# fgarciacardenas/SplaTAM

Hardware: AMD Instinct MI355X
Metric: rasterize fwd+bwd frames/sec @640×480, 300k Gaussians; HBM GB/s vs peak (higher is better)
Workload: dtype f32

## Files before the change

### splatam_amd/csrc/gsr_backward.hip

```cpp
#include <cstdlib>
#include <utility>

#include "gsr_chain.h"
#include "gsr_diag.h"
#include "gsr_glue_common.h"
#include "gsr_render_fwd.h"

namespace gsr {

template <bool OPAC>
__device__ __forceinline__ void pair_geom(float* vk, float araw, float dLa, float G, v2f d) {
    if constexpr (OPAC) {
        const v2f ho = v2f{araw, G} * dLa;
        const v2f hv = ho.x * d;
        const v2f hh = hv.x * d;
        vk[0] = hv.x;
        vk[1] = hv.y;
        vk[2] = hh.x;
        vk[3] = hh.y;
        vk[4] = hv.y * d.y;
        vk[5] = ho.y;
        return;
    }
    const v2f hv = (araw * dLa) * d;
// ... 370 lines not shown
                    e[k].dx = d[k].x;
                    e[k].dy = d[k].y;
                    e[k].xx = d[k].x * d[k].x;
                    e[k].xy = d[k].x * d[k].y;
                    e[k].yy = d[k].y * d[k].y;
                    e[k].o2 = o * o;
                    e[k].c2 = dch[k] * dch[k];
                    const float hc = h * dch[k];
                    e[k].hc[0] = hc * dp0;
                    e[k].hc[1] = hc * dp1;
                    e[k].hc[2] = hc * dp2;
                }
                mom_pass<MOM, 0, 4>(e, mdp2, mdpp, lane, dst);
                mom_pass<MOM, 4, 4>(e, mdp2, mdpp, lane, dst);
                mom_pass<MOM, 8, 4>(e, mdp2, mdpp, lane, dst);
                if constexpr (MOM == 1) {
                    mom_pass<MOM, 12, 4>(e, mdp2, mdpp, lane, dst);
                } else {
                    mom_pass<MOM, 12, 4>(e, mdp2, mdpp, lane, dst);
                    mom_pass<MOM, 16, 4>(e, mdp2, mdpp, lane, dst);
                    mom_pass<MOM, 20, 4>(e, mdp2, mdpp, lane, dst);
                    mom_pass<MOM, 24, 5>(e, mdp2, mdpp, lane, dst);
                    mom_pass<MOM, 29, 5>(e, mdp2, mdpp, lane, dst);
                }
            } else if constexpr (NV <= 6) {
                float v[4 * NV];
#pragma unroll
                for (int k = 0; k < 4; k++) {
                    pair_geom<OPAC>(v + NV * k, araw[k], dLa[k], G[k], d[k]);
                    pair_colours<COL1, COL2, Q2, C1>(v + NV * k + O_C1, dch[k], dp01, dp2, dq0, dq01, dq2);
                }
                if constexpr (kAblate == 1) {
#pragma unroll
                    for (int q = 0; q < 4 * NV; q++) ablate_sink += v[q];
                } else {
                    reduce_store<NV>(v, lane, dst, true);
                }
            } else {
                constexpr int NA = 5 + (OPAC ? 1 : 0), NB = NV - NA;
                {
                    float v[4 * NA];
#pragma unroll
                    for (int k = 0; k < 4; k++) pair_geom<OPAC>(v + NA * k, araw[k], dLa[k], G[k], d[k]);
                    reduce_store<NA>(v, lane, dst, true);
                }
                {
                    float v[4 * NB];
#pragma unroll
                    for (int k = 0; k < 4; k++) {
                        pair_colours<COL1, COL2, Q2, C1>(v + NB * k, dch[k], dp01, dp2, dq0, dq01, dq2);
                    }
                    reduce_store<NB>(v, lane, dst + NA, true);
                }
            }
        }
        dg.phase(3);
        __syncthreads();
        dg.phase(4);
        constexpr int TPE = TILE_PIX / BB, NQ = (NV + TPE - 1) / TPE, NQR = (RS + TPE - 1) / TPE;
        int t_ = tid;
        asm volatile("" : "+v"(t_));
        const int e = t_ / TPE, q = t_ % TPE;
        if (kAblate != 2 && e < cnt) {
            float c[NQ];
#pragma unroll
            for (int i = 0; i < NQ; i++) c[i] = 0.f;
            const int nb = __popc((uint32_t)s_mask[e]);
            float* src = s_acc + (int)s_base[e] * NV;
            for (int b = 0; b < nb; b++, src += NV) {
#pragma unroll
                for (int i = 0; i < NQ; i++)
                    if (q + TPE * i < NV) {
                        c[i] += src[q + TPE * i];
                        if constexpr (!kBulkClear) src[q + TPE * i] = 0.f;
                    }
            }
            float* dst = inst + (size_t)RS * s_u[e];
#pragma unroll
            for (int i = 0; i < NQR; i++)
                if (q + TPE * i < RS) {
                    const float val = i < NQ ? c[i] : 0.f;
                    dst[q + TPE * i] = val;
                }
        }
        dg.phase(5);
        __syncthreads();
        if constexpr (kBulkClear) {
            const int used = cnt > 0 ? (int)s_base[cnt - 1] + __popc((uint32_t)s_mask[cnt - 1]) : 0;
            float4* const a4 = reinterpret_cast<float4*>(s_acc);
            const float4 z = make_float4(0.f, 0.f, 0.f, 0.f);
            for (int q4 = tid; q4 < (used * NV + 3) / 4; q4 += TILE_PIX) a4[q4] = z;
        }
        dg.phase(6);
        dg.batch();
        hi -= cnt;
    }
    if (kAblate == 1 && ablate_sink == 1.2345f) inst[0] = ablate_sink;
}

template <bool DUAL, bool OPAC, bool COL1, bool COL2, int Q2 = 3, int MOM = 0>
__global__ void __launch_bounds__(TILE_PIX, (bwd_waves<DUAL, OPAC, COL1, COL2, Q2, MOM>()))
render_bwd_kernel(Camera cam, const uint2* __restrict__ ranges, const PointEntry* __restrict__ point_list,
                  const float4* __restrict__ rr, const uint32_t* __restrict__ blocksums,
                  const float* __restrict__ final_T,
                  const uint32_t* __restrict__ n_contrib, const float* __restrict__ dL_dpix,
                  const float* __restrict__ dL_dpix2, float* __restrict__ inst, BwdGuard guard,
                  unsigned long long* clk) {
    kclock_begin(clk);
    RenderDiag dg;
    dg.begin();
    if (guard.overflow()) {
        kclock_end(clk);
        return;
    }
    __shared__ __attribute__((aligned(16))) char smem[BwdShape<DUAL, OPAC, COL1, COL2, Q2, MOM>::bytes];
    const int tid = threadIdx.x;
    const int tile = sched_tile(cam), tx = tile % cam.gx, ty = tile / cam.gx;
    dg.tile(tile);
    const int px = tx * TILE_X + tile_px(tid);
    const int py = ty * TILE_Y + tile_py(tid);
    const bool inside = px < cam.W && py < cam.H;
    const int pid = py * cam.W + px;
    const int HW = cam.W * cam.H;
    BwdPix pin{0.f, 0u, 0.f, 0.f, 0.f, 0.f, 0.f, 0.f};
    if (inside) {
        pin.T_final = final_T[pid];
        pin.last = n_contrib[pid];
        pin.dp0 = dL_dpix[pid];
        pin.dp1 = dL_dpix[HW + pid];
        pin.dp2 = dL_dpix[2 * HW + pid];
        if (DUAL) {
            pin.dq0 = dL_dpix2[pid];
            if (Q2 == 3) {
                pin.dq1 = dL_dpix2[HW + pid];
                pin.dq2 = dL_dpix2[2 * HW + pid];
            }
        }
    }
    if constexpr (!DUAL && COL1 && MOM == 0) {
        if (!__syncthreads_or(pin.dp1 != 0.f || pin.dp2 != 0.f)) {
            bwd_tile<DUAL, OPAC, COL1, COL2, Q2, MOM, 1>(cam, tile, pin, ranges, point_list, rr, blocksums, inst, guard,
                                                         smem, dg);
            dg.end();
            kclock_end(clk);
            return;
        }
    }
    bwd_tile<DUAL, OPAC, COL1, COL2, Q2, MOM>(cam, tile, pin, ranges, point_list, rr, blocksums, inst, guard, smem, dg);
    dg.end();
    kclock_end(clk);
}

constexpr size_t track_lds_bytes() {
    return FwdShape<true>::bytes > BwdShape<true, false, false, true, 1, 0>::bytes
               ? FwdShape<true>::bytes
               : BwdShape<true, false, false, true, 1, 0>::bytes;
}
template <bool IMAGES>
__global__ void __launch_bounds__(TILE_PIX, 5)
render_track_kernel(Camera cam, const uint2* __restrict__ ranges, PointEntry* __restrict__ point_list,
                    uint64_t* __restrict__ keys, const float4* __restrict__ rr, const uint32_t* __restrict__ blocksums,
                    float* __restrict__ final_T, uint32_t* __restrict__ n_contrib, float* __restrict__ out_color,
                    float* __restrict__ out_color2, float* __restrict__ out_depth, SpecGuard guard,
                    unsigned long long* clk, TrackL1 l1, float* __restrict__ inst) {
    kclock_begin(clk);
    RenderDiag dg;
    dg.begin();
    if (guard.overflow()) {
        kclock_end(clk);
        return;
    }
    __shared__ __attribute__((aligned(16))) char smem[track_lds_bytes()];
    if constexpr (!IMAGES) {
        final_T = nullptr;
        cam.rowmax = nullptr;
    }
    const int tile = sched_tile(cam);
    dg.tile(tile);
    const FwdPix f = fwd_tile<true>(cam, tile, ranges, point_list, keys, rr, guard, smem, dg);
    float grad[4];
    constexpr bool kStoreGrads = false;
    static_assert(!kStoreGrads, "render_track_kernel's callers pass no gradient images");
    fwd_epilogue<true, true, kStoreGrads>(cam, tile, f, final_T, n_contrib, out_color, out_color2, out_depth, l1,
                                          grad);
    __syncthreads();
    const BwdPix pin{f.T, f.last16 >> 4, grad[0], grad[1], grad[2], grad[3], 0.f, 0.f};
    Camera cb = cam;
    cb.rowmax = nullptr;
    bwd_tile<true, false, false, true, 1, 0>(cb, tile, pin, ranges, point_list, rr, blocksums, inst,
                                             BwdGuard{guard.counters, guard.cap_inst}, smem, dg);
    dg.end();
    kclock_end(clk);
}

int track_records_stride() { return BwdShape<true, false, false, true, 1, 0>::RS; }

hipError_t launch_render_track(const Camera& cam, const uint2* ranges, uint64_t* point_list, uint64_t* keys,
                               GeomPtrs geo, float* final_T, uint32_t* n_contrib, float* out_color,
                               float* out_color2, float* out_depth, SpecGuard guard, const TrackL1& l1, float* inst,
                               hipStream_t s, unsigned long long* clk) {
    auto k = final_T != nullptr ? render_track_kernel<true> : render_track_kernel<false>;
    hipLaunchKernelGGL(k, dim3(cam.gx * cam.gy), dim3(TILE_PIX), 0, s, cam, ranges, point_list,
                       keys, geo.rr, geo.blocksums, final_T, n_contrib, out_color, out_color2, out_depth, guard, clk,
                       l1, inst);
    return hipGetLastError();
}

template <bool DUAL, bool OPAC, bool COL1, bool COL2, int Q2 = 3>
static auto bwd_variant() { return render_bwd_kernel<DUAL, OPAC, COL1, COL2, Q2>; }

RecLayout bwd_rec_layout(unsigned need, bool dual) {
    const bool op = need & NEED_OPACITY, c1 = need & NEED_COLORS, c2 = dual && (need & NEED_COLORS2);
    const int q2 = (dual && (need & NEED_DL2_CH0_ONLY)) ? 1 : 3;
    RecLayout L;
    int nv = 5;
    L.o_op = op ? nv : -1;
    nv += op ? 1 : 0;
    L.o_c1 = c1 ? nv : -1;
    nv += c1 ? 3 : 0;
    L.o_c2 = c2 ? nv : -1;
    L.n_c2 = c2 ? q2 : 0;
    nv += L.n_c2;
    L.stride = (nv + 1) & ~1;
    return L;
}

hipError_t launch_render_bwd(const Camera& cam, const uint2* ranges, const uint64_t* point_list, GeomPtrs geo,
                             const float* final_T, const uint32_t* n_contrib, const float* dL_dpix,
                             const float* colors2, const float* dL_dpix2, unsigned need, float* inst,
                             BwdGuard guard, hipStream_t s, unsigned long long* clk) {
    const bool op = need & NEED_OPACITY, c1 = need & NEED_COLORS, c2 = colors2 && (need & NEED_COLORS2);
    const bool q1 = need & NEED_DL2_CH0_ONLY;
    auto k = bwd_variant<false, true, true, false>();
    if (!colors2) {
        k = op ? (c1 ? bwd_variant<false, 1, 1, 0>() : bwd_variant<false, 1, 0, 0>())
               : (c1 ? bwd_variant<false, 0, 1, 0>() : bwd_variant<false, 0, 0, 0>());
    } else if (q1 && !op && !c1) {
        k = c2 ? bwd_variant<true, 0, 0, 1, 1>() : bwd_variant<true, 0, 0, 0, 1>();
    } else if (q1) {
        k = op ? (c1 ? (c2 ? bwd_variant<true, 1, 1, 1, 1>() : bwd_variant<true, 1, 1, 0, 1>())
                     : (c2 ? bwd_variant<true, 1, 0, 1, 1>() : bwd_variant<true, 1, 0, 0, 1>()))
               : (c2 ? bwd_variant<true, 0, 1, 1, 1>() : bwd_variant<true, 0, 1, 0, 1>());
    } else {
        k = op ? (c1 ? (c2 ? bwd_variant<true, 1, 1, 1>() : bwd_variant<true, 1, 1, 0>())
                     : (c2 ? bwd_variant<true, 1, 0, 1>() : bwd_variant<true, 1, 0, 0>()))
               : (c1 ? (c2 ? bwd_variant<true, 0, 1, 1>() : bwd_variant<true, 0, 1, 0>())
                     : (c2 ? bwd_variant<true, 0, 0, 1>() : bwd_variant<true, 0, 0, 0>()));
    }
    hipLaunchKernelGGL(k, dim3(cam.gx * cam.gy), dim3(TILE_PIX), 0, s, cam, ranges, point_list, geo.rr, geo.blocksums,
                       final_T, n_contrib, dL_dpix, dL_dpix2, inst, guard, clk);
    return hipGetLastError();
}

template <bool POSE, bool SHL>
__device__ __forceinline__ void gauss_bwd_body(Camera cam, GaussIn g, GeomPtrs geo, const int* __restrict__ radii,
                                               const float* __restrict__ inst, RecLayout rec, GradsOut out,
                                               BwdGuard guard, PoseFuse pf) {
    if constexpr (!SHL) {
        g.shs = nullptr;
        g.M = 0;
    }
    const int i = blockIdx.x * blockDim.x + threadIdx.x;
    if (!POSE && i >= g.P) return;
    const bool live = i < g.P;
    const int nsh = g.shs ? (cam.sh_degree + 1) * (cam.sh_degree + 1) : 0;
    float g2[9] = {0.f, 0.f, 0.f, 0.f, 0.f, 0.f, 0.f, 0.f, 0.f};
    float dcol2[3] = {0.f, 0.f, 0.f};
    float dmean[3] = {0.f, 0.f, 0.f}, dcov[6] = {0.f, 0.f, 0.f, 0.f, 0.f, 0.f}, dscale[3] = {0.f, 0.f, 0.f},
          drot[4] = {0.f, 0.f, 0.f, 0.f};
    float dsh[48];
#pragma unroll
    for (int k = 0; k < 48; k++) dsh[k] = 0.f;
    GaussGeom gg;
    gg.m = make_float3(0.f, 0.f, 0.f);
    gg.s = make_float3(0.f, 0.f, 0.f);
    gg.q = make_float4(0.f, 0.f, 0.f, 0.f);
    const int rad = live ? radii[i] : 0;
    const bool xf_geom = POSE && pf.ls;
    TrackXf x;
    x.mw = pf.means_world; x.ur = pf.unnorm_rot; x.ls = pf.ls; x.scols = pf.scols;
    XfRaw xr{};
    if (xf_geom && live) xr = track_xform_load(x, i, false);
    uint32_t off = 0, cnt = 0, tl = 0xFFFFFFFFu;
    if (POSE && live && rad > 0) {
        off = geo.offsets[i];
        cnt = geo.tiles[i];
        tl = reinterpret_cast<const uint32_t*>(geo.bin)[4 * (size_t)i + 3];
    }
    __shared__ Pose s_pose;
    if constexpr (POSE) {
        if (pf.ls || pf.scols != 1) {
            if (threadIdx.x == 0) s_pose = make_pose(pf.cam_q, pf.cam_t, pf.qs);
            __syncthreads();
        }
    }
    if (live && (POSE || rad > 0)) {
        if (xf_geom) {
            const Pose ps = s_pose;
            float m[3], sv[3];
            track_xform_geom_raw(xr, x.scols, ps, m, gg.q, sv);
            gg.m = make_float3(m[0], m[1], m[2]);
            gg.s = make_float3(sv[0], sv[1], sv[2]);
        } else {
            gg = load_geom(g, i);
        }
    }
    if (live && rad > 0 && !guard.overflow()) {
        if (!POSE) {
            off = geo.offsets[i];
            cnt = geo.tiles[i];
            tl = reinterpret_cast<const uint32_t*>(geo.bin)[4 * (size_t)i + 3];
        }
        float acc[INST_REC_MAX];
#pragma unroll
        for (int m = 0; m < INST_REC_MAX; m++) acc[m] = 0.f;
        const int np = rec.stride / 2;
        constexpr int RU = 4;
        for (uint32_t e0 = 0; e0 < cnt; e0 += RU) {
            float2 v[RU][INST_REC_MAX / 2];
#pragma unroll
            for (int k = 0; k < RU; k++) {
                const float2* r = reinterpret_cast<const float2*>(inst + (size_t)rec.stride * (off + e0 + k));
#pragma unroll
                for (int m = 0; m < INST_REC_MAX / 2; m++)
                    v[k][m] = (m < np && e0 + k < cnt && tile_live(tl, e0 + k)) ? r[m] : make_float2(0.f, 0.f);
            }
#pragma unroll
            for (int k = 0; k < RU; k++)
                if (e0 + k < cnt && tile_live(tl, e0 + k)) {
#pragma unroll
                    for (int m = 0; m < INST_REC_MAX / 2; m++)
                        if (m < np) {
// ... 379 lines not shown
```

### splatam_amd/csrc/gsr_capi.hip

```cpp
#include <cstdio>
#include <cstdlib>
#include <cstring>
#include <algorithm>
#include <atomic>
#include <string>

#include "../../include/gsr.h"
#include "../../include/gsr_glue.h"
#include "gsr_host.h"

using namespace gsr;

namespace {
thread_local std::string g_last_error;

__global__ void zero_words_kernel(uint32_t* __restrict__ p, size_t n) {
    for (size_t k = blockIdx.x * (size_t)blockDim.x + threadIdx.x; k < n; k += (size_t)gridDim.x * blockDim.x) p[k] = 0u;
}
std::atomic<int> g_cus[kMaxDevices];
}

namespace gsr {
int fail(int code, const std::string& msg) {
    g_last_error = msg;
// ... 53 lines not shown
    uint32_t* p = nullptr;
    uint32_t* dp = nullptr;
    hipEvent_t ev = nullptr;
    ~Pinned() {
        if (p) (void)hipHostFree(p);
        if (ev) (void)hipEventDestroy(ev);
    }
    int ensure(int dev) {
        hipError_t e;
        if (!p) {
            if ((e = hipHostMalloc((void**)&p, 32,
                                   hipHostMallocMapped | hipHostMallocCoherent | hipHostMallocPortable)) != hipSuccess)
                return hip_fail(e, "hipHostMalloc");
            if ((e = hipHostGetDevicePointer((void**)&dp, p, 0)) != hipSuccess)
                return hip_fail(e, "hipHostGetDevicePointer");
        }
        if (!ev) {
            int cur = 0;
            (void)hipGetDevice(&cur);
            if (cur != dev) (void)hipSetDevice(dev);
            e = hipEventCreateWithFlags(&ev, hipEventDisableTiming);
            if (cur != dev) (void)hipSetDevice(cur);
            if (e != hipSuccess) return hip_fail(e, "hipEventCreate");
        }
        return GSR_OK;
    }
};
thread_local Pinned g_pinned[kMaxDevices];
const bool g_snap_copy = getenv("GSR_SNAP_COPY") && atoi(getenv("GSR_SNAP_COPY")) != 0;
struct RatioHint {
    std::atomic<double> v{3.0};
};
RatioHint g_inst_ratio[kMaxDevices];

Camera make_camera(const gsr_settings* s) {
    Camera c;
    c.W = s->image_width;
    c.H = s->image_height;
    c.tan_fovx = s->tan_fovx;
    c.tan_fovy = s->tan_fovy;
    c.focal_y = (float)c.H / (2.0f * s->tan_fovy);
    c.focal_x = (float)c.W / (2.0f * s->tan_fovx);
    c.gx = (c.W + TILE_X - 1) / TILE_X;
    c.gy = (c.H + TILE_Y - 1) / TILE_Y;
    c.view = s->viewmatrix;
    c.proj = s->projmatrix;
    c.campos = s->campos;
    c.bg = s->bg;
    c.scale_modifier = s->scale_modifier;
    c.sh_degree = s->sh_degree;
    c.prefiltered = s->prefiltered;
    return c;
}

GaussIn make_gauss(const gsr_gaussians* g) {
    GaussIn o;
    o.P = g->P;
    o.M = g->shs ? g->M : 0;
    o.means3D = g->means3D;
    o.shs = (g->shs && g->M > 0) ? g->shs : nullptr;
    o.colors = g->colors_precomp;
    o.opacities = g->opacities;
    o.scales = g->scales;
    o.rotations = g->rotations;
    o.cov3D = g->cov3D_precomp;
    o.colors2 = nullptr;
    o.sh_staged = 0;
    o.alive = nullptr;
    return o;
}

int validate(const gsr_settings* s, const gsr_gaussians* g, bool forward) {
    if (!s || !g) return fail(GSR_ERR_INVALID_ARG, "null settings or gaussians");
    if (g->P < 0) return fail(GSR_ERR_INVALID_ARG, "P must be >= 0");
    if (s->binning != GSR_BINNING_CULLED && s->binning != GSR_BINNING_REFERENCE)
        return fail(GSR_ERR_INVALID_ARG, "settings.binning must be GSR_BINNING_CULLED or GSR_BINNING_REFERENCE");
    if (s->image_width <= 0 || s->image_height <= 0) return fail(GSR_ERR_INVALID_ARG, "image size must be positive");
    if (s->image_width > 16 * 65535 || s->image_height > 16 * 65535)
        return fail(GSR_ERR_INVALID_ARG, "image too large for 16-bit tile coordinates");
    if (g->P == 0) return GSR_OK;
    if (!g->means3D) return fail(GSR_ERR_INVALID_ARG, "means3D is required");
    if (forward && !g->opacities) return fail(GSR_ERR_INVALID_ARG, "opacities are required");
    if (!s->viewmatrix || !s->projmatrix || !s->bg) return fail(GSR_ERR_INVALID_ARG, "camera matrices / bg missing");
    const bool has_sh = g->shs && g->M > 0;
    if (!g->colors_precomp && !has_sh)
        return fail(GSR_ERR_INVALID_ARG, "Please provide excatly one of either SHs or precomputed colors!");
    if (!g->colors_precomp && !s->campos) return fail(GSR_ERR_INVALID_ARG, "campos required for SH colours");
    if (has_sh && (s->sh_degree < 0 || s->sh_degree > 3 || (s->sh_degree + 1) * (s->sh_degree + 1) > g->M))
        return fail(GSR_ERR_INVALID_ARG, "sh_degree must be in [0,3] with (deg+1)^2 <= M");
    const bool has_sr = g->scales && g->rotations;
    if (!has_sr && !g->cov3D_precomp)
        return fail(GSR_ERR_INVALID_ARG,
                    "Please provide exactly one of either scale/rotation pair or precomputed 3D covariance!");
    return GSR_OK;
}

template <class T>
int obtain(gsr_alloc_fn alloc, void* ctx, int kind, size_t bytes, const char* what, T** out) {
    *out = (T*)alloc(ctx, kind, bytes);
    return *out ? GSR_OK : fail(GSR_ERR_ALLOC, std::string("allocator returned NULL (") + what + ")");
}

struct ReuseIn {
    EqualPairs pairs;
    int prev_num_rendered;
    const void* prev_geom;
    void* prev_binning;
    void* prev_image;
    const int* prev_radii;
    int* reused;
};

struct FwdCall {
    const gsr_settings* settings = nullptr;
    const gsr_gaussians* gaussians = nullptr;
    const float* colors2 = nullptr;
    float* out_color = nullptr;
    float* out_color2 = nullptr;
    float* out_depth = nullptr;
    int* radii = nullptr;
    gsr_alloc_fn alloc = nullptr;
    void* alloc_ctx = nullptr;
    void* stream = nullptr;
    int capacity = 0;
    uint32_t* status = nullptr;
    const TrackL1* l1 = nullptr;
    const TrackXf* xf = nullptr;
    float* track_inst = nullptr;
    const uint8_t* alive = nullptr;
    const ReuseIn* reuse = nullptr;
};

FwdCall fwd_call(const gsr_settings* settings, const gsr_gaussians* gaussians, float* out_color, float* out_depth,
                 int* radii, gsr_alloc_fn alloc, void* alloc_ctx, void* stream) {
    FwdCall c;
    c.settings = settings; c.gaussians = gaussians;
    c.out_color = out_color; c.out_depth = out_depth; c.radii = radii;
    c.alloc = alloc; c.alloc_ctx = alloc_ctx; c.stream = stream;
    return c;
}
FwdCall& dual(FwdCall& c, const float* colors2, float* out_color2) {
    c.colors2 = colors2; c.out_color2 = out_color2;
    return c;
}
FwdCall& statics(FwdCall& c, int capacity, uint32_t* status) {
    c.capacity = capacity; c.status = status;
    return c;
}

bool stores_no_images(const FwdCall& c) { return c.track_inst && !c.out_color && !c.out_color2 && !c.out_depth; }

int check_forward(const FwdCall& c) {
    const int rc = validate(c.settings, c.gaussians, true);
    if (c.track_inst && (!c.l1 || !c.colors2 || c.capacity <= 0))
        return fail(GSR_ERR_INVALID_ARG, "the fused render backward needs the static dual forward with the L1 loss");
    if (rc != GSR_OK) return rc;
    if (!c.alloc) return fail(GSR_ERR_INVALID_ARG, "allocator callback required");
    if (!stores_no_images(c)) {
        if (!c.out_color || !c.out_depth) return fail(GSR_ERR_INVALID_ARG, "output image pointers required");
        if (c.colors2 && !c.out_color2) return fail(GSR_ERR_INVALID_ARG, "out_color2 required with colors2");
    }
    if (c.colors2 && c.gaussians->P > 0 && !c.gaussians->means3D)
        return fail(GSR_ERR_INVALID_ARG, "means3D is required");
    return GSR_OK;
}

struct Forward {
    const FwdCall& c;
    hipStream_t stream;
    int dev;
    Pinned& pin;
    Camera cam;
    GaussIn g;
    int P, W, H, ntiles;
    GeomLayout GL;
    ImgLayout IL;
    void* geom = nullptr;
    GeomPtrs geo{};
    ImgPtrs img{};
    uint32_t* cursor = nullptr;
    bool lds_hist;
    uint32_t* cmat = nullptr;
    uint32_t* tile_tot = nullptr;
    bool force_radix;
    bool scan_in_duplicate;
    bool eager;
    bool gated = false;
    Gate eq_gate;
    uint32_t epoch = 0;
    uint32_t cap = 0;

    static bool force_radix_env() {
        static const bool on = getenv("GSR_FORCE_RADIX") && atoi(getenv("GSR_FORCE_RADIX")) != 0;
        return on;
    }
    explicit Forward(const FwdCall& call)
        : c(call), stream((hipStream_t)call.stream), dev(stream_device(stream)), pin(g_pinned[dev]),
          cam(make_camera(call.settings)), g(make_gauss(call.gaussians)), P(g.P), W(cam.W), H(cam.H),
          ntiles(cam.gx * cam.gy), GL(GeomLayout::make(P)), IL(ImgLayout::make(W, H)),
          lds_hist(ntiles <= MAX_LDS_TILES), force_radix(force_radix_env() && call.capacity <= 0),
          scan_in_duplicate(lds_hist && !force_radix), eager(call.capacity <= 0) {
        g.colors2 = c.colors2;
        g.alive = c.alive;
        if (c.xf) g.xf = *c.xf;
        cam.pre_shift = GL.shift;
        cam.cull = c.settings->binning != GSR_BINNING_REFERENCE ? 1 : 0;
        cam.tail_exact = eager ? 1 : 0;
    }
    uint32_t* status() const { return eager ? nullptr : c.status; }
    template <class T>
    int obtain(int kind, size_t bytes, const char* what, T** out) {
        return ::obtain(c.alloc, c.alloc_ctx, kind, bytes, what, out);
    }

    int setup_buffers() {
        void* image = nullptr;
        geom = c.alloc(c.alloc_ctx, GSR_BUF_GEOM, GL.total);
        image = c.alloc(c.alloc_ctx, GSR_BUF_IMAGE, IL.total);
        if (!geom || !image) return fail(GSR_ERR_ALLOC, "allocator returned NULL (geom/image buffer)");
        geo = GeomPtrs::at(geom, GL);
        img = ImgPtrs::at(image, IL);
        bind_schedule(cam, img, dev);
        cursor = img.tile_count + (size_t)ntiles * TILE_CTR_STRIDE;
        hipError_t e;
        if (lds_hist && P > 0) {
            if (int rc = obtain(GSR_BUF_SCRATCH, 4 * ((size_t)GL.nb * ntiles + ntiles), "tile count matrix", &cmat))
                return rc;
            tile_tot = cmat + (size_t)GL.nb * ntiles;
        } else if ((e = zero_async(img.tile_count, 8 * (size_t)ntiles * TILE_CTR_STRIDE, stream)) != hipSuccess) {
            return hip_fail(e, "memset tile counts");
        }
        if (c.reuse && c.reuse->reused) *c.reuse->reused = 0;
        return GSR_OK;
    }

    int empty_map() {
        hipError_t e;
        if ((e = zero_async(img.ranges, sizeof(uint2) * (size_t)ntiles, stream)) != hipSuccess)
            return hip_fail(e, "memset ranges");
        void* bin;
        if (int rc = obtain(GSR_BUF_BINNING, BinLayout::make(0, W, H).total, "binning buffer", &bin)) return rc;
        const size_t img3 = sizeof(float) * 3 * (size_t)W * H;
        if (const TrackL1* l1 = c.l1) {
            if ((e = zero_async(l1->loss, sizeof(float), stream)) != hipSuccess ||
                (l1->terms && (e = zero_async(l1->terms, 2 * sizeof(float), stream)) != hipSuccess) ||
                (l1->dL_dim && (e = zero_async(l1->dL_dim, img3, stream)) != hipSuccess) ||
                (l1->dL_dds && (e = zero_async(l1->dL_dds, img3, stream)) != hipSuccess))
                return hip_fail(e, "zero loss");
        }
        if (stores_no_images(c)) return 0;
        if ((e = zero_async(c.out_color, img3, stream)) != hipSuccess ||
            (e = zero_async(c.out_depth, sizeof(float) * (size_t)W * H, stream)) != hipSuccess ||
            (c.colors2 && (e = zero_async(c.out_color2, img3, stream)) != hipSuccess))
            return hip_fail(e, "zero outputs");
        return 0;
    }

    int gate_on_comparison() {
        gated = c.reuse && eager && !c.colors2 && !c.track_inst && !c.l1 && !c.xf && lds_hist && !force_radix &&
                !sh_staged(cam, g);
        if (!gated) return GSR_OK;
        static std::atomic<uint32_t> g_epoch{0};
        do epoch = g_epoch.fetch_add(1u, std::memory_order_relaxed) + 1u; while (epoch == 0u);
        uint32_t* word = geo.counters + 5;
        hipError_t e;
        if ((e = launch_epoch_mismatch(c.reuse->pairs, word, epoch, stream)) != hipSuccess)
            return hip_fail(e, "geometry comparison");
        cam.gate = Gate{word, epoch, 1u};
        eq_gate = Gate{word, epoch, 0u};
        if ((e = launch_reuse_copy(eq_gate, c.reuse->prev_geom, geom, GL.counters, GL.tiles, g.colors,
                                   c.reuse->prev_radii, c.radii, P, stream)) != hipSuccess)
            return hip_fail(e, "geometry reuse");
        return GSR_OK;
    }

    int snapshot_counters(bool stored_by_kernel) {
        if (int rc = pin.ensure(dev)) return rc;
        hipError_t e;
        if (!stored_by_kernel &&
            (e = hipMemcpyAsync(pin.p, geo.counters, 32, hipMemcpyDeviceToHost, stream)) != hipSuccess)
            return hip_fail(e, "copy num_rendered");
        if ((e = hipEventRecord(pin.ev, stream)) != hipSuccess) return hip_fail(e, "record num_rendered");
        return GSR_OK;
    }

    int counts_and_ranges() {
        hipError_t e;
        if (!scan_in_duplicate && (e = launch_identity_order(img.order, ntiles, stream)) != hipSuccess)
            return hip_fail(e, "render schedule");
        if (!c.radii) return fail(GSR_ERR_INVALID_ARG, "radii output required");
        {
            StageTimer t(GSR_STAGE_PREPROCESS, P, stream, true);
            if (sh_staged(cam, g)) {
                if ((e = launch_sh_eval(cam, g, geo, stream)) != hipSuccess) return hip_fail(e, "sh_eval");
                g.sh_staged = 1;
            }
            if ((e = launch_preprocess(cam, g, geo, c.radii, lds_hist ? cmat : img.tile_count, lds_hist, ntiles,
                                       GL.nb, stream, t.kclock())) != hipSuccess)
                return hip_fail(e, "preprocess");
        }
        {
            StageTimer t(GSR_STAGE_RANGES, ntiles, stream, lds_hist);
            if (lds_hist) {
                if ((e = launch_tile_colscan(cmat, GL.nb, ntiles, tile_tot, geo, img.ranges, status(),
                                             !scan_in_duplicate, stream, t.kclock(), cam.gate)) != hipSuccess)
                    return hip_fail(e, "tile count scan");
            } else if ((e = launch_scan_counts(geo, GL.nb, img.tile_count, TILE_CTR_STRIDE, ntiles, img.ranges,
                                               status(), stream)) != hipSuccess) {
// ... 801 lines not shown
```

### splatam_amd/csrc/gsr_render_fwd.h

```cpp
#pragma once
#include "gsr_common.h"
#include "gsr_diag.h"

namespace gsr {

constexpr int TILE_SORT_THREADS = 256;
constexpr uint32_t TILE_SORT_REGS = 1024;

template <int M>
__device__ __forceinline__ uint32_t lane_xor(uint32_t x) {
    static_assert(M == 1 || M == 2 || M == 4 || M == 8 || M == 16 || M == 32, "lane xor distance");
    if constexpr (M == 1) {
        return (uint32_t)__builtin_amdgcn_mov_dpp((int)x, 0xB1, 0xF, 0xF, false);
    } else if constexpr (M == 2) {
        return (uint32_t)__builtin_amdgcn_mov_dpp((int)x, 0x4E, 0xF, 0xF, false);
    } else if constexpr (M == 4) {
        const uint32_t up = (uint32_t)__builtin_amdgcn_mov_dpp((int)x, 0x104, 0xF, 0xF, false);
        const uint32_t dn = (uint32_t)__builtin_amdgcn_mov_dpp((int)x, 0x114, 0xF, 0xF, false);
        return (__lane_id() & 4) ? dn : up;
    } else if constexpr (M == 8) {
        return (uint32_t)__builtin_amdgcn_mov_dpp((int)x, 0x128, 0xF, 0xF, false);
    } else if constexpr (M == 16) {
        const auto p = __builtin_amdgcn_permlane16_swap(x, x, false, false);
        return (__lane_id() & 16) ? p[0] : p[1];
    } else {
        const auto p = __builtin_amdgcn_permlane32_swap(x, x, false, false);
        return (__lane_id() & 32) ? p[0] : p[1];
    }
}
template <int M>
__device__ __forceinline__ uint64_t lane_xor64(uint64_t v) {
    return ((uint64_t)lane_xor<M>((uint32_t)(v >> 32)) << 32) | lane_xor<M>((uint32_t)v);
}

template <int E, int J>
__device__ __forceinline__ void bitonic_reg_stage(uint64_t (&v)[E], uint32_t base, uint32_t k) {
#pragma unroll
    for (int e = 0; e < E; e++) {
        if (e & J) continue;
        const bool up = ((base + (uint32_t)e) & k) == 0;
        const uint64_t a = v[e], b = v[e + J];
        const bool sw = (b < a) == up;
        v[e] = sw ? b : a;
        v[e + J] = sw ? a : b;
    }
}

__device__ __forceinline__ uint64_t bitonic_pick(uint64_t v, uint64_t o, bool keep_min) {
    return ((o < v) == keep_min) ? o : v;
}

template <int E, int LK, int LJ>
__device__ __forceinline__ void bitonic_net(uint64_t (&v)[E], uint32_t base, uint64_t* sk) {
    constexpr uint32_t k = 1u << LK, j = 1u << LJ;
    if constexpr (j >= (uint32_t)E) {
        const bool up = (base & k) == 0, keep_min = ((base & j) == 0) == up;
        if constexpr (j >= 64u * E) {
#pragma unroll
            for (int e = 0; e < E; e++) sk[base + e] = v[e];
            __syncthreads();
#pragma unroll
            for (int e = 0; e < E; e++) v[e] = bitonic_pick(v[e], sk[(base + e) ^ j], keep_min);
            __syncthreads();
        } else {
#pragma unroll
            for (int e = 0; e < E; e++) v[e] = bitonic_pick(v[e], lane_xor64<(int)(j / E)>(v[e]), keep_min);
        }
    } else {
        bitonic_reg_stage<E, (int)j>(v, base, k);
    }
    constexpr int LOGN = E == 1 ? 8 : E == 2 ? 9 : 10;
    if constexpr (LJ > 0) bitonic_net<E, LK, LJ - 1>(v, base, sk);
    else if constexpr (LK < LOGN) bitonic_net<E, LK + 1, LK>(v, base, sk);
}

template <int E, typename Emit>
__device__ void tile_sort_regs(const uint64_t* __restrict__ src, uint32_t cnt, Emit emit, uint64_t* sk) {
    static_assert(E == 1 || E == 2 || E == 4, "256 x E keys");
    const uint32_t base = threadIdx.x * E;
    uint64_t v[E];
#pragma unroll
    for (int e = 0; e < E; e++) v[e] = base + e < cnt ? src[base + e] : ~0ull;
    bitonic_net<E, 1, 0>(v, base, sk);
#pragma unroll
    for (int e = 0; e < E; e++)
        if (base + e < cnt) emit(base + e, v[e] == ~0ull ? 0u : (uint32_t)v[e]);
}

#if GSR_FWD_ABLATE == 7
static __device__ uint16_t g_fab_mask[1u << 23];
#endif
__device__ __forceinline__ void tile_sort_bucket(uint64_t* __restrict__ src, uint32_t cnt,
                                                 PointEntry* __restrict__ dst, uint64_t* sk) {
    auto emit = [&](uint32_t i, uint32_t gi) { dst[i] = (PointEntry)gi; };
    if (GSR_FWD_ABLATE == 1) {
        for (uint32_t i = threadIdx.x; i < cnt; i += TILE_SORT_THREADS) emit(i, (uint32_t)src[i]);
        return;
    }
    if (cnt <= 1) {
        if (cnt == 1 && threadIdx.x == 0) emit(0, (uint32_t)src[0]);
        return;
    }
    if (cnt <= 256) {
        tile_sort_regs<1>(src, cnt, emit, sk);
        return;
    }
    if (cnt <= 512) {
        tile_sort_regs<2>(src, cnt, emit, sk);
        return;
    }
    const uint32_t nch = (cnt + TILE_SORT_REGS - 1) / TILE_SORT_REGS;
    const uint32_t base = threadIdx.x * 4;
    for (uint32_t c = 0; c < nch; c++) {
        const uint32_t c0 = c * TILE_SORT_REGS, len = min(TILE_SORT_REGS, cnt - c0);
        uint64_t v[4];
#pragma unroll
        for (int e = 0; e < 4; e++) v[e] = base + e < len ? src[c0 + base + e] : ~0ull;
        bitonic_net<4, 1, 0>(v, base, sk);
#pragma unroll
        for (int e = 0; e < 4; e++) {
            if (base + e >= len) continue;
            if (nch == 1) emit(base + e, v[e] == ~0ull ? 0u : (uint32_t)v[e]);
            else src[c0 + base + e] = v[e];
        }
    }
    if (nch == 1) return;
    __syncthreads();
    for (uint32_t c = 0; c < nch; c++) {
        const uint32_t c0 = c * TILE_SORT_REGS, len = min(TILE_SORT_REGS, cnt - c0);
        uint64_t v[4];
        uint32_t pos[4];
#pragma unroll
        for (int e = 0; e < 4; e++) {
            v[e] = base + e < len ? src[c0 + base + e] : ~0ull;
            pos[e] = base + e;
        }
        for (uint32_t c2 = 0; c2 < nch; c2++) {
            if (c2 == c) continue;
            const uint32_t d0 = c2 * TILE_SORT_REGS, dlen = min(TILE_SORT_REGS, cnt - d0);
            __syncthreads();
            for (uint32_t i = threadIdx.x; i < dlen; i += TILE_SORT_THREADS) sk[i] = src[d0 + i];
            __syncthreads();
#pragma unroll
            for (int e = 0; e < 4; e++) {
                uint32_t lo = 0;
#pragma unroll
                for (uint32_t st = TILE_SORT_REGS; st > 0; st >>= 1)
                    if (lo + st <= dlen && sk[lo + st - 1] < v[e]) lo += st;
                pos[e] += lo;
            }
        }
#pragma unroll
        for (int e = 0; e < 4; e++)
            if (base + e < len) emit(pos[e], (uint32_t)v[e]);
    }
    __syncthreads();
}

template <bool DUAL>
struct FwdShape {
    static constexpr int LS = RENDER_BATCH + 4;
    static constexpr size_t o_ab = 0, o_c = o_ab + 2 * 16 * (RENDER_BATCH + 1), o_d = o_c + 16 * (RENDER_BATCH + 1);
    static constexpr size_t o_list = o_d + 16 * (DUAL ? RENDER_BATCH + 1 : 1);
    static constexpr size_t o_mask = o_list + 2 * 16 * LS;
    static constexpr size_t bytes = o_mask + 2 * RENDER_BATCH;
    static_assert(2 * 16 * (RENDER_BATCH + 1) >= TILE_SORT_REGS * sizeof(uint64_t) && TILE_SORT_THREADS == TILE_PIX,
                  "tile sort (256 x 4 keys) LDS aliases s_a / s_b");
};

struct FwdPix {
    float T, C2, C5, D;
    v2f C01, C34;
    uint32_t last16;
};

template <bool DUAL>
__device__ __forceinline__ FwdPix fwd_tile(const Camera& cam, int tile, const uint2* __restrict__ ranges,
                                           PointEntry* __restrict__ point_list, uint64_t* __restrict__ keys,
                                           const float4* __restrict__ rr, const SpecGuard& guard, char* smem,
                                           RenderDiag& dg) {
    using L = FwdShape<DUAL>;
    constexpr int LS = L::LS;
    float4* const s_ab = reinterpret_cast<float4*>(smem + L::o_ab);
    float4* const s_a = s_ab;
    float4* const s_b = s_ab + RENDER_BATCH + 1;
    float4* const s_c = reinterpret_cast<float4*>(smem + L::o_c);
    [[maybe_unused]] float4* const s_d = reinterpret_cast<float4*>(smem + L::o_d);
    uint16_t* const s_mask = reinterpret_cast<uint16_t*>(smem + L::o_mask);
    uint16_t* const s_list = reinterpret_cast<uint16_t*>(smem + L::o_list);
    const int tid = threadIdx.x, w = tid >> 6, row = (tid >> 4) & 3;
    const int tx = tile % cam.gx, ty = tile / cam.gx;
    const int px = tx * TILE_X + tile_px(tid);
    const int py = ty * TILE_Y + tile_py(tid);
    const float x0 = (float)(tx * TILE_X), y0 = (float)(ty * TILE_Y);
    const bool inside = px < cam.W && py < cam.H;
    const v2f pix = v2f{(float)px, (float)py};
    const uint2 range = ranges[tile];
    bool done = !inside;
    float T = 1.f, C2 = 0.f, D = 15.0f;
    float C5 = 0.f;
    v2f C01 = v2f{0.f, 0.f}, C34 = v2f{0.f, 0.f};
    uint32_t last16 = 0;
    float4 pa = make_float4(0.f, 0.f, 0.f, 0.f), pb = pa, pc = pa, pd = pa;
    uint32_t pg = 0, pgn = 0;
    if (keys != nullptr) {
        tile_sort_bucket(keys + range.x, range.y - range.x, point_list + range.x,
                         reinterpret_cast<uint64_t*>(s_ab));
        __syncthreads();
        if constexpr (kDupPhase == 1) {
            tile_sort_bucket(keys + range.x, range.y - range.x, point_list + range.x,
                             reinterpret_cast<uint64_t*>(s_ab));
            __syncthreads();
        }
    }
    if (tid == 0) {
        s_a[RENDER_BATCH] = pa;
        s_b[RENDER_BATCH] = pa;
        s_c[RENDER_BATCH] = pa;
        if (DUAL) s_d[RENDER_BATCH] = pa;
    }
    auto fetch_id = [&](uint32_t s0) {
        if (s0 + tid < range.y) pgn = pe_id(point_list[s0 + tid]);
    };
    auto fetch_rec = [&](uint32_t s0) {
        if (s0 + tid < range.y) {
            pg = pgn;
            const RenderRec r = load_rr(rr, pg);
            pa = r.q0; pb = r.q1; pc = r.q2;
            if (DUAL) pd = r.q3;
        }
    };
    fetch_id(range.x);
    fetch_rec(range.x);
    fetch_id(range.x + RENDER_BATCH);
    const uint32_t mean4 = sched_mean4(cam, guard.counters);
    const bool multi_round = sched_multi_round(cam);
    dg.phase(0);
    for (uint32_t start = range.x; start < range.y; start += RENDER_BATCH) {
        prio_by_remaining((int)(range.y - start), mean4, multi_round);
        if (__syncthreads_and(done)) break;
        const int cnt = (int)min((uint32_t)RENDER_BATCH, range.y - start);
        PointEntry ent = 0;
        if (tid < cnt) {
            float xs = x0, ys = y0;
            asm volatile("" : "+v"(xs), "+v"(ys));
            uint32_t pm = GSR_FWD_ABLATE == 5 ? block_mask(pa, pb, xs, ys)
                        : GSR_FWD_ABLATE == 6 ? 0xFFFFu : 0u;
#if GSR_FWD_ABLATE == 7
            pm = g_fab_mask[start + tid];
            if (pm == 0u) {
                pm = block_mask_exact(pa, pb, xs, ys);
                g_fab_mask[start + tid] = (uint16_t)pm;
            }
#else
            if (GSR_FWD_ABLATE != 5 && GSR_FWD_ABLATE != 6) pm = block_mask_exact(pa, pb, xs, ys);
#endif
            s_a[tid] = pa;
            s_b[tid] = pb;
            s_c[tid] = DUAL ? make_float4(pc.x, pc.y, pc.z, pd.z) : pc;
            if (DUAL) s_d[tid] = pd;
            s_mask[tid] = (uint16_t)pm;
            ent = ((PointEntry)pm << 32) | pg;
        }
        __syncthreads();
        dg.phase(1);
        fetch_rec(start + RENDER_BATCH);
        fetch_id(start + 2 * RENDER_BATCH);
        if (tid < cnt) point_list[start + tid] = ent;
        const int jmin0[4] = {0, 0, 0, 0};
        static_assert(16 * RENDER_BATCH < 65536, "16-bit byte offsets");
        int n = build_row_lists(s_mask, cnt, w, jmin0, s_list + 4 * w * LS, LS, (uint16_t)(16 * RENDER_BATCH), 16u);
        if constexpr (kDupPhase == 2) {
            asm volatile("" ::: "memory");
            n = build_row_lists(s_mask, cnt, w, jmin0, s_list + 4 * w * LS, LS, (uint16_t)(16 * RENDER_BATCH), 16u);
        }
        const uint16_t* my_list = s_list + (4 * w + row) * LS;
        const uint32_t pos16 = 16u * (start - range.x) + 16u;
        dg.phase(2);
        for (int i = 0; i < (GSR_FWD_ABLATE == 2 ? 0 : n); i += 4) {
            if (done) break;
            int jb[4];
#pragma unroll
            for (int k = 0; k < 4; k++)
                jb[k] = (int)((const volatile __attribute__((address_space(3))) uint16_t*)my_list)[i + k];
            auto rec = [&](const float4* arr, int k) {
                return *reinterpret_cast<const float4*>(reinterpret_cast<const char*>(arr) + jb[k]);
            };
            float alpha[4], depth[4];
            bool ok[4];
#pragma unroll
            for (int k = 0; k < 4; k++) {
                const float4 a = rec(s_a, k), b = rec(s_b, k);
                const float p2 = eval_p2(a, b, pix_delta(a, pix));
                alpha[k] = fminf(0.99f, b.y * __builtin_amdgcn_exp2f(p2));
                depth[k] = b.z;
                ok[k] = p2 <= 0.0f && alpha[k] >= 1.0f / 255.0f;
            }
#pragma unroll
            for (int k = 0; k < 4; k++) {
                const bool okk = ok[k] && !done;
                const float test_T = T * (1.f - alpha[k]);
                const bool term = okk && test_T < 0.0001f;
                done = done || term;
                const bool blend = okk && !term;
                const float4 c = rec(s_c, k);
                float4 c2;
                if (DUAL) c2 = rec(s_d, k);
                if (blend) {
                    const float wgt = alpha[k] * T;
                    C01 = __builtin_elementwise_fma(v2f{c.x, c.y}, v2f{wgt, wgt}, C01);
                    if (DUAL) {
                        const v2f c25 = __builtin_elementwise_fma(v2f{c.z, c.w}, v2f{wgt, wgt}, v2f{C2, C5});
                        C2 = c25.x;
                        C5 = c25.y;
                        C34 = __builtin_elementwise_fma(v2f{c2.x, c2.y}, v2f{wgt, wgt}, C34);
                    } else {
                        C2 += c.z * wgt;
                    }
                    if (T > 0.5f && test_T < 0.5f) D = depth[k];
                    T = test_T;
                    last16 = pos16 + (uint32_t)jb[k];
                }
            }
        }
        dg.phase(3);
        __syncthreads();
        dg.phase(4);
        dg.batch();
    }
    return FwdPix{T, C2, C5, D, C01, C34, last16};
}


#ifndef GSR_L1_CH
#define GSR_L1_CH 8
#endif

__device__ __forceinline__ void l1_finish(const TrackL1& l1) {
    if constexpr (kAblate == 6) return;
    __shared__ float s_fin[16];
    const int tid = threadIdx.x, w = tid >> 6, lane = tid & 63, row4 = lane >> 4;
    const int nb = gridDim.x * gridDim.y;
    if (last_block_arrive_grouped(scratch_counters(l1.scratch))) {
        float v[4] = {0.f, 0.f, 0.f, 0.f}, r[1];
        {
            float v2[2] = {0.f, 0.f};
            gather_partials<2, GSR_L1_CH>(scratch_partials(l1.scratch), 2, nb, tid, TILE_PIX, v2);
            v[0] = v2[0];
            v[1] = v2[1];
        }
        wave_reduce_n<4>(v, r);
        if ((lane & 15) == 0) s_fin[w * 4 + row4] = r[0];
        __syncthreads();
        if (tid == 0) {
            const float s0 = (s_fin[0] + s_fin[4]) + (s_fin[8] + s_fin[12]);
            const float s1 = (s_fin[1] + s_fin[5]) + (s_fin[9] + s_fin[13]);
            l1.loss[0] = l1.w_im * s0 + l1.w_depth * s1;
            if (l1.terms) {
                l1.terms[0] = l1.w_im * s0;
                l1.terms[1] = l1.w_depth * s1;
            }
        }
    }
}

template <bool DUAL, bool L1, bool STORE_GRADS, bool L1_FINISH = true>
__device__ __forceinline__ void fwd_epilogue(const Camera& cam, int tile, const FwdPix& f, float* __restrict__ final_T,
                                             uint32_t* __restrict__ n_contrib, float* __restrict__ out_color,
                                             float* __restrict__ out_color2, float* __restrict__ out_depth,
                                             const TrackL1& l1, float (&grad)[4]) {
    const int tid = threadIdx.x, w = tid >> 6, row = (tid >> 4) & 3;
    const int tx = tile % cam.gx, ty = tile / cam.gx;
    const int px = tx * TILE_X + tile_px(tid);
    const int py = ty * TILE_Y + tile_py(tid);
    const bool inside = px < cam.W && py < cam.H;
    const float T = f.T, C2 = f.C2, C5 = f.C5, D = f.D;
    const float C0 = f.C01.x, C1 = f.C01.y, C3 = f.C34.x, C4 = f.C34.y;
    const uint32_t last16 = f.last16;
    (void)C3; (void)C4; (void)C5;
#pragma unroll
    for (int c = 0; c < 4; c++) grad[c] = 0.f;
    if (cam.rowmax) {
        uint32_t rmax = last16 >> 4;
#pragma unroll
        for (int o = 8; o > 0; o >>= 1) rmax = max(rmax, (uint32_t)__shfl_xor((int)rmax, o));
        if ((tid & 15) == 0) cam.rowmax[16 * tile + 4 * w + row] = rmax;
    }
    float l1_seed = 0.f, l1_gd = 0.f, l1_gi[3] = {0.f, 0.f, 0.f};
    if constexpr (L1 && GSR_FWD_ABLATE != 4) {
        if (inside) {
            const int pid = py * cam.W + px;
            const int HW = cam.W * cam.H;
            l1_seed = l1.seed[0];
            l1_gd = l1.gt_depth[pid];
#pragma unroll
            for (int c = 0; c < 3; c++) l1_gi[c] = l1.gt_im[c * HW + pid];
        }
    }
    if (inside && final_T != nullptr && (GSR_FWD_ABLATE != 8 || T == 1.2345f)) {
        const int pid = py * cam.W + px;
        const int HW = cam.W * cam.H;
        auto st = [](float* p, float v) { *p = v; };
        st(final_T + pid, T);
        n_contrib[pid] = last16 >> 4;
        st(out_color + pid, C0 + T * cam.bg[0]);
        st(out_color + HW + pid, C1 + T * cam.bg[1]);
        st(out_color + 2 * HW + pid, C2 + T * cam.bg[2]);
        st(out_depth + pid, D);
        if (DUAL) {
            st(out_color2 + pid, C3 + T * cam.bg[0]);
            st(out_color2 + HW + pid, C4 + T * cam.bg[1]);
            st(out_color2 + 2 * HW + pid, C5 + T * cam.bg[2]);
        }
    }
    if constexpr (L1 && GSR_FWD_ABLATE != 4) {
        __shared__ float s_red[4 * 4];
        __shared__ float s_tot[4];
        float v[4] = {0.f, 0.f, 0.f, 0.f};
        if (inside) {
            const int pid = py * cam.W + px;
            const int HW = cam.W * cam.H;
            const float g = l1_seed;
            const float im[3] = {C0 + T * cam.bg[0], C1 + T * cam.bg[1], C2 + T * cam.bg[2]};
            const float d = C3 + T * cam.bg[0], sil = C4 + T * cam.bg[1], dsq = C5 + T * cam.bg[2];
            const float gd = l1_gd;
            const float unc = dsq - d * d;
            const bool m = gd > 0.f && !isnan(d) && !isnan(unc) && sil > l1.sil_thres;
            const float gi[3] = {l1_gi[0], l1_gi[1], l1_gi[2]};
            if (m) {
                v[0] = fabsf(gi[0] - im[0]) + fabsf(gi[1] - im[1]) + fabsf(gi[2] - im[2]);
                v[1] = fabsf(gd - d);
            }
#pragma unroll
            for (int c = 0; c < 3; c++) {
                const float x = gi[c] - im[c];
                grad[c] = m ? (g * l1.w_im) * (x > 0.f ? -1.f : (x < 0.f ? 1.f : 0.f)) : 0.f;
            }
            const float xd = gd - d;
            grad[3] = m ? (g * l1.w_depth) * (xd > 0.f ? -1.f : (xd < 0.f ? 1.f : 0.f)) : 0.f;
            if (STORE_GRADS) {
#pragma unroll
                for (int c = 0; c < 3; c++) l1.dL_dim[c * HW + pid] = grad[c];
                l1.dL_dds[pid] = grad[3];
                l1.dL_dds[HW + pid] = 0.f;
                l1.dL_dds[2 * HW + pid] = 0.f;
            }
        }
        float r[1];
        wave_reduce_n<4>(v, r);
        const int lane = tid & 63, row4 = lane >> 4;
        if ((lane & 15) == 0) s_red[w * 4 + row4] = r[0];
        __syncthreads();
        if (tid < 4) s_tot[tid] = (s_red[tid] + s_red[4 + tid]) + (s_red[8 + tid] + s_red[12 + tid]);
        __syncthreads();
        if (tid < 2) st_agent(scratch_partials(l1.scratch) + 2 * tile + tid, s_tot[tid]);
        if (L1_FINISH) l1_finish(l1);
    }
}

}
```

Baseline: 6647.

## Pack second color channel into spare slot and add mid-size tile sort path

In the fused track kernel's forward walk, the dual-color record's needed channel is packed into the unused w lane of the s_b record, and a constant 1.0 replaces the second channel. This drops the s_d LDS array, cutting LDS footprint and per-pair LDS reads. A new sort path for tiles of 513-768 entries sorts a 512 block and a 256 block in registers, then merges them with a binary-search merge instead of the chunked general path. The packing relies on callers using the transform-fused forward where that channel is known to be 1, and validation is tightened to require it.

After: 6682 (median of 6 runs). No clear change (+0.5%).

```diff
diff --git a/splatam_amd/csrc/gsr_backward.hip b/splatam_amd/csrc/gsr_backward.hip
--- a/splatam_amd/csrc/gsr_backward.hip
+++ b/splatam_amd/csrc/gsr_backward.hip
@@ -546,8 +546,8 @@
 }
 
 constexpr size_t track_lds_bytes() {
-    return FwdShape<true>::bytes > BwdShape<true, false, false, true, 1, 0>::bytes
-               ? FwdShape<true>::bytes
+    return FwdShape<true, true>::bytes > BwdShape<true, false, false, true, 1, 0>::bytes
+               ? FwdShape<true, true>::bytes
                : BwdShape<true, false, false, true, 1, 0>::bytes;
 }
 template <bool IMAGES>
@@ -571,7 +571,7 @@
     }
     const int tile = sched_tile(cam);
     dg.tile(tile);
-    const FwdPix f = fwd_tile<true>(cam, tile, ranges, point_list, keys, rr, guard, smem, dg);
+    const FwdPix f = fwd_tile<true, true>(cam, tile, ranges, point_list, keys, rr, guard, smem, dg);
     float grad[4];
     constexpr bool kStoreGrads = false;
     static_assert(!kStoreGrads, "render_track_kernel's callers pass no gradient images");
diff --git a/splatam_amd/csrc/gsr_capi.hip b/splatam_amd/csrc/gsr_capi.hip
--- a/splatam_amd/csrc/gsr_capi.hip
+++ b/splatam_amd/csrc/gsr_capi.hip
@@ -229,8 +229,9 @@
 
 int check_forward(const FwdCall& c) {
     const int rc = validate(c.settings, c.gaussians, true);
-    if (c.track_inst && (!c.l1 || !c.colors2 || c.capacity <= 0))
-        return fail(GSR_ERR_INVALID_ARG, "the fused render backward needs the static dual forward with the L1 loss");
+    if (c.track_inst && (!c.l1 || !c.colors2 || !c.xf || c.capacity <= 0))
+        return fail(GSR_ERR_INVALID_ARG,
+                    "the fused render backward needs the static, transform-fused dual forward with the L1 loss");
     if (rc != GSR_OK) return rc;
     if (!c.alloc) return fail(GSR_ERR_INVALID_ARG, "allocator callback required");
     if (!stores_no_images(c)) {
diff --git a/splatam_amd/csrc/gsr_render_fwd.h b/splatam_amd/csrc/gsr_render_fwd.h
--- a/splatam_amd/csrc/gsr_render_fwd.h
+++ b/splatam_amd/csrc/gsr_render_fwd.h
@@ -6,6 +6,7 @@
 
 constexpr int TILE_SORT_THREADS = 256;
 constexpr uint32_t TILE_SORT_REGS = 1024;
+constexpr uint32_t TILE_SORT_SPLIT = 768;
 
 template <int M>
 __device__ __forceinline__ uint32_t lane_xor(uint32_t x) {
@@ -109,6 +110,32 @@
         tile_sort_regs<2>(src, cnt, emit, sk);
         return;
     }
+    if (cnt <= TILE_SORT_SPLIT) {
+        const uint32_t t = threadIdx.x;
+        uint64_t v[2], u[1];
+#pragma unroll
+        for (int e = 0; e < 2; e++) v[e] = src[2 * t + e];
+        u[0] = 512u + t < cnt ? src[512u + t] : ~0ull;
+        bitonic_net<2, 1, 0>(v, 2 * t, sk);
+        bitonic_net<1, 1, 0>(u, t, sk);
+        sk[2 * t] = v[0];
+        sk[2 * t + 1] = v[1];
+        sk[512u + t] = u[0];
+        __syncthreads();
+        uint32_t lo[3] = {0u, 0u, 0u};
+#pragma unroll
+        for (uint32_t st = 512; st > 0; st >>= 1) {
+#pragma unroll
+            for (int e = 0; e < 2; e++)
+                if (lo[e] + st <= 256u && sk[512u + lo[e] + st - 1] < v[e]) lo[e] += st;
+            if (lo[2] + st <= 512u && sk[lo[2] + st - 1] < u[0]) lo[2] += st;
+        }
+#pragma unroll
+        for (int e = 0; e < 2; e++) emit(2 * t + e + lo[e], (uint32_t)v[e]);
+        if (512u + t < cnt) emit(t + lo[2], (uint32_t)u[0]);
+        __syncthreads();
+        return;
+    }
     const uint32_t nch = (cnt + TILE_SORT_REGS - 1) / TILE_SORT_REGS;
     const uint32_t base = threadIdx.x * 4;
     for (uint32_t c = 0; c < nch; c++) {
@@ -157,11 +184,11 @@
     __syncthreads();
 }
 
-template <bool DUAL>
+template <bool DUAL, bool C2_ZONE = false>
 struct FwdShape {
     static constexpr int LS = RENDER_BATCH + 4;
     static constexpr size_t o_ab = 0, o_c = o_ab + 2 * 16 * (RENDER_BATCH + 1), o_d = o_c + 16 * (RENDER_BATCH + 1);
-    static constexpr size_t o_list = o_d + 16 * (DUAL ? RENDER_BATCH + 1 : 1);
+    static constexpr size_t o_list = o_d + 16 * ((DUAL && !C2_ZONE) ? RENDER_BATCH + 1 : 1);
     static constexpr size_t o_mask = o_list + 2 * 16 * LS;
     static constexpr size_t bytes = o_mask + 2 * RENDER_BATCH;
     static_assert(2 * 16 * (RENDER_BATCH + 1) >= TILE_SORT_REGS * sizeof(uint64_t) && TILE_SORT_THREADS == TILE_PIX,
@@ -174,13 +201,15 @@
     uint32_t last16;
 };
 
-template <bool DUAL>
+template <bool DUAL, bool C2_ZONE = false>
 __device__ __forceinline__ FwdPix fwd_tile(const Camera& cam, int tile, const uint2* __restrict__ ranges,
                                            PointEntry* __restrict__ point_list, uint64_t* __restrict__ keys,
                                            const float4* __restrict__ rr, const SpecGuard& guard, char* smem,
                                            RenderDiag& dg) {
-    using L = FwdShape<DUAL>;
+    static_assert(DUAL || !C2_ZONE, "C2_ZONE is a form of the dual walk");
+    using L = FwdShape<DUAL, C2_ZONE>;
     constexpr int LS = L::LS;
+    constexpr bool REC_D = DUAL && !C2_ZONE;
     float4* const s_ab = reinterpret_cast<float4*>(smem + L::o_ab);
     float4* const s_a = s_ab;
     float4* const s_b = s_ab + RENDER_BATCH + 1;
@@ -217,7 +246,7 @@
         s_a[RENDER_BATCH] = pa;
         s_b[RENDER_BATCH] = pa;
         s_c[RENDER_BATCH] = pa;
-        if (DUAL) s_d[RENDER_BATCH] = pa;
+        if (REC_D) s_d[RENDER_BATCH] = pa;
     }
     auto fetch_id = [&](uint32_t s0) {
         if (s0 + tid < range.y) pgn = pe_id(point_list[s0 + tid]);
@@ -256,9 +285,9 @@
             if (GSR_FWD_ABLATE != 5 && GSR_FWD_ABLATE != 6) pm = block_mask_exact(pa, pb, xs, ys);
 #endif
             s_a[tid] = pa;
-            s_b[tid] = pb;
+            s_b[tid] = C2_ZONE ? make_float4(pb.x, pb.y, pb.z, pd.x) : pb;
             s_c[tid] = DUAL ? make_float4(pc.x, pc.y, pc.z, pd.z) : pc;
-            if (DUAL) s_d[tid] = pd;
+            if (REC_D) s_d[tid] = pd;
             s_mask[tid] = (uint16_t)pm;
             ent = ((PointEntry)pm << 32) | pg;
         }
@@ -287,6 +316,7 @@
                 return *reinterpret_cast<const float4*>(reinterpret_cast<const char*>(arr) + jb[k]);
             };
             float alpha[4], depth[4];
+            [[maybe_unused]] float c3[4];
             bool ok[4];
 #pragma unroll
             for (int k = 0; k < 4; k++) {
@@ -294,6 +324,7 @@
                 const float p2 = eval_p2(a, b, pix_delta(a, pix));
                 alpha[k] = fminf(0.99f, b.y * __builtin_amdgcn_exp2f(p2));
                 depth[k] = b.z;
+                if (C2_ZONE) c3[k] = b.w;
                 ok[k] = p2 <= 0.0f && alpha[k] >= 1.0f / 255.0f;
             }
 #pragma unroll
@@ -304,8 +335,13 @@
                 done = done || term;
                 const bool blend = okk && !term;
                 const float4 c = rec(s_c, k);
-                float4 c2;
-                if (DUAL) c2 = rec(s_d, k);
+                v2f c34 = v2f{0.f, 0.f};
+                if (C2_ZONE) {
+                    c34 = v2f{c3[k], 1.0f};
+                } else if (DUAL) {
+                    const float4 c2 = rec(s_d, k);
+                    c34 = v2f{c2.x, c2.y};
+                }
                 if (blend) {
                     const float wgt = alpha[k] * T;
                     C01 = __builtin_elementwise_fma(v2f{c.x, c.y}, v2f{wgt, wgt}, C01);
@@ -313,7 +349,7 @@
                         const v2f c25 = __builtin_elementwise_fma(v2f{c.z, c.w}, v2f{wgt, wgt}, v2f{C2, C5});
                         C2 = c25.x;
                         C5 = c25.y;
-                        C34 = __builtin_elementwise_fma(v2f{c2.x, c2.y}, v2f{wgt, wgt}, C34);
+                        C34 = __builtin_elementwise_fma(c34, v2f{wgt, wgt}, C34);
                     } else {
                         C2 += c.z * wgt;
                     }
```
